# yycho0108/qpwcnet

Hardware: AMD Instinct MI355X
Metric: image-pairs/sec at 256x512 fp32 (higher is better)
Workload: dtype f32; 1 GPU; BASELINE configs[1]: full 6-level PWC-Net (qpwcnet build_flower) inference, batch 8 per GPU, 256x512 fp32, channels_last, d=4 cost volume + WarpV2; global_batch=8, batch_per_gpu=8, parallelism=dp1 (pairs sharded, RCCL all-gather of the 6 per-level EPE), hipgraph=True

## Files before the change

### qpwcnet_amd/csrc/encoder.hip

```cpp
#include "common.h"

namespace qpwc {

__device__ __forceinline__ float enc_mishf(float x) {
    const float e = __builtin_amdgcn_exp2f(fminf(x, 20.0f) * 1.4426950408889634f);
    const float t = e * (e + 2.0f);
    const float m = x * (t * __builtin_amdgcn_rcpf(t + 2.0f));
    return m;
}

typedef float f32x4e __attribute__((ext_vector_type(4)));

__device__ __forceinline__ float2 ld2(const float* p) { return *reinterpret_cast<const float2*>(p); }
__device__ __forceinline__ float2 ld2(const __half* p) { return __half22float2(*reinterpret_cast<const __half2*>(p)); }
__device__ __forceinline__ void st4q(float* p, float4 v) { *reinterpret_cast<float4*>(p) = v; }
__device__ __forceinline__ void st4q(__half* p, float4 v) {
    __half2 lo = __floats2half2_rn(v.x, v.y), hi = __floats2half2_rn(v.z, v.w);
    uint2 u;
    u.x = *reinterpret_cast<unsigned*>(&lo);
    u.y = *reinterpret_cast<unsigned*>(&hi);
    *reinterpret_cast<uint2*>(p) = u;
}

constexpr int kEcTH = 8, kEcTW = 16;
constexpr int kEcHW = kEcTW + 2, kEcNH = (kEcTH + 2) * kEcHW;

template <int C>
__device__ __forceinline__ int ec_slot(int q, int hp) {
    return C == 16 ? (q ^ ((hp >> 2) & 3)) : (q ^ ((hp >> 1) & (C / 4 - 1)));
}

#ifndef QPWC_ENC_NT
#define QPWC_ENC_NT 1
#endif
#ifndef QPWC_UPCONV16_NFB_MIN_WGS
#define QPWC_UPCONV16_NFB_MIN_WGS 512
#endif
#ifndef QPWC_UPCONV256_TH
#define QPWC_UPCONV256_TH 2
#endif
#ifndef QPWC_UPCONV128_TH
#define QPWC_UPCONV128_TH 4
#endif
#ifndef QPWC_UPCONV64_LDS_TOTAL
#define QPWC_UPCONV64_LDS_TOTAL 82944
#endif
#ifndef QPWC_W_NEXT_ALWAYS
#define QPWC_W_NEXT_ALWAYS 1
#endif
#ifndef QPWC_W_NEXT_ALWAYS_F16
#define QPWC_W_NEXT_ALWAYS_F16 0
#endif
#if QPWC_W_NEXT_ALWAYS
#define QPWC_LOAD_W_NEXT(END) load_w(wn, kb + 1 < (END) ? kb + 1 : kb)
#else
#define QPWC_LOAD_W_NEXT(END) do { if (kb + 1 < (END)) load_w(wn, kb + 1); } while (0)
#endif
#ifdef QPWC_ENC_STAMP
__device__ long long g_enc_census[4096 * 6];
#define ENC_CENSUS(i) do { if (census_on) census_p[i] = __builtin_amdgcn_s_memtime(); } while (0)
#else
#define ENC_CENSUS(i) do { } while (0)
#endif
template <int C, int NT>
__global__ __launch_bounds__(256, 4) void conv3x3_mish_kernel(const float* __restrict__ x,
                                                              const float* __restrict__ weight,
                                                              const float* __restrict__ bias,
                                                              float* __restrict__ out, int H, int W,
                                                              int pad_h, int pad_w, int tiles_x, int tiles_y,
                                                              int groups_x) {
    constexpr int NQ = C / 4;
    constexpr int NFT = C / 16;
    constexpr int NKC = C / 16;
    constexpr int NLD = (kEcNH * NQ + 255) / 256;
    constexpr int NBUF = NT > 1 ? 2 : 1;
    __shared__ __attribute__((aligned(16))) float in_s[NBUF * kEcNH * C];
    const int tid0 = threadIdx.x;
    const int wave = __builtin_amdgcn_readfirstlane(tid0 >> 6);
    const int lane = tid0 & 63, n0 = lane & 15, g0 = lane >> 4;
    const int grp = xcd_swizzle(blockIdx.x, gridDim.x);
    const int gx0 = grp % groups_x, ty = (grp / groups_x) % tiles_y, b = grp / (groups_x * tiles_y);
    const int tx0 = gx0 * NT;
    const int Y0 = ty * kEcTH;
    const float* xb = x + (int64_t)b * H * W * C;
    const int Ho = H + pad_h, Wo = W + pad_w;
    float* ob = out + (int64_t)b * Ho * Wo * C;

    auto stage_load = [&](int tid, int tx, float4 (&v)[NLD]) {
        const int X0 = tx * kEcTW;
#pragma unroll
        for (int it = 0; it < NLD; ++it) {
            const int idx = tid + 256 * it;
            const int hp = idx / NQ, q = idx - hp * NQ;
            const int hy = hp / kEcHW, hx = hp - hy * kEcHW;
            const int gy = Y0 - 1 + hy, gx = X0 - 1 + hx;
            v[it] = (idx < kEcNH * NQ && gy >= 0 && gy < H && gx >= 0 && gx < W)
                        ? *reinterpret_cast<const float4*>(xb + ((int64_t)gy * W + gx) * C + 4 * q)
                        : make_float4(0.f, 0.f, 0.f, 0.f);
        }
    };
    auto stage_write = [&](int tid, int buf, const float4 (&v)[NLD]) {
#pragma unroll
        for (int it = 0; it < NLD; ++it) {
            const int idx = tid + 256 * it;
            const int hp = idx / NQ, q = idx - hp * NQ;
            if (idx < kEcNH * NQ)
                *reinterpret_cast<float4*>(in_s + buf * (kEcNH * C) + hp * C + 4 * ec_slot<C>(q, hp)) = v[it];
        }
    };
#ifdef QPWC_ENC_STAMP
    const bool census_on = tid0 == 0 && blockIdx.x < 4096;
    long long* census_p = g_enc_census + (blockIdx.x < 4096 ? blockIdx.x : 0) * 6;
    if (census_on)
        census_p[5] = (long long)(unsigned)__builtin_amdgcn_s_getreg((4) | (0 << 6) | (31 << 11)) |
                      ((long long)(unsigned)__builtin_amdgcn_s_getreg((20) | (0 << 6) | (31 << 11)) << 32);
#endif
    ENC_CENSUS(0);
    float4 st[NLD];
    stage_load(tid0, tx0, st);
#ifdef QPWC_ENC_STAMP
    asm volatile("s_waitcnt vmcnt(0)" ::: "memory");
#endif
    ENC_CENSUS(1);
    stage_write(tid0, 0, st);
    __syncthreads();
    ENC_CENSUS(2);

#pragma unroll 1
    for (int t = 0; t < NT; ++t) {
        const int tx = tx0 + t;
        if (tx >= tiles_x) break;
        const bool more = t + 1 < NT && tx + 1 < tiles_x;

        const int X0 = tx * kEcTW;
        const float* tile_s = in_s + (t & (NBUF - 1)) * (kEcNH * C);
        const float* wt = weight;
        int n = n0, g = g0, tid = tid0;
        if (NT > 1) asm volatile("" : "+r"(wt), "+v"(n), "+v"(g), "+v"(tid));
        if (more) stage_load(tid, tx + 1, st);
#pragma unroll
        for (int ft = 0; ft < NFT; ++ft) {
            f32x4e wld[9][NKC];
#pragma unroll
            for (int k = 0; k < 9; ++k)
#pragma unroll
                for (int kc = 0; kc < NKC; ++kc)
                    wld[k][kc] = *reinterpret_cast<const f32x4e*>(wt + ((int64_t)k * C + 16 * ft + n) * C + 16 * kc + 4 * g);
            f32x4e acc[2];
            acc[0] = f32x4e{0.f, 0.f, 0.f, 0.f};
            acc[1] = f32x4e{0.f, 0.f, 0.f, 0.f};
#pragma unroll
            for (int ky = 0; ky < 3; ++ky)
#pragma unroll
                for (int kx = 0; kx < 3; ++kx)
#pragma unroll
                    for (int kc = 0; kc < NKC; ++kc) {
                        f32x4e bv[2];
#pragma unroll
                        for (int m = 0; m < 2; ++m) {
                            const int hp = (2 * wave + m + ky) * kEcHW + n + kx;
                            const int q = 4 * kc + g;
                            const int slot = ec_slot<C>(q, hp);
                            bv[m] = *reinterpret_cast<const f32x4e*>(tile_s + hp * C + 4 * slot);
                        }
#pragma unroll
                        for (int tt = 0; tt < 4; ++tt)
#pragma unroll
                            for (int m = 0; m < 2; ++m)
                                acc[m] = __builtin_amdgcn_mfma_f32_16x16x4f32(wld[ky * 3 + kx][kc][tt], bv[m][tt], acc[m], 0, 0, 0);
                    }
            if (ft == NFT - 1) ENC_CENSUS(3);
            const float4 bq = *reinterpret_cast<const float4*>(bias + 16 * ft + 4 * g);
#pragma unroll
            for (int m = 0; m < 2; ++m) {
                const int gy = Y0 + 2 * wave + m, gx = X0 + n;
                if (gy < H && gx < W)
                    *reinterpret_cast<float4*>(ob + ((int64_t)gy * Wo + gx) * C + 16 * ft + 4 * g) =
                        make_float4(enc_mishf(acc[m][0] + bq.x), enc_mishf(acc[m][1] + bq.y),
                                    enc_mishf(acc[m][2] + bq.z), enc_mishf(acc[m][3] + bq.w));
            }
        }
        if (pad_w > 0 && X0 + kEcTW >= W) {
            for (int i = tid; i < kEcTH * pad_w * NQ; i += 256) {
                const int q = i % NQ, r = i / NQ, col = r % pad_w, row = r / pad_w;
                const int gy = Y0 + row;
                if (gy < H) *reinterpret_cast<float4*>(ob + ((int64_t)gy * Wo + W + col) * C + 4 * q) = make_float4(0.f, 0.f, 0.f, 0.f);
            }
        }
        if (pad_h > 0 && Y0 + kEcTH >= H) {
            const int x_end = (X0 + kEcTW >= W) ? Wo : X0 + kEcTW;
            for (int i = tid; i < pad_h * (x_end - X0) * NQ; i += 256) {
                const int q = i % NQ, r = i / NQ, col = r % (x_end - X0), row = r / (x_end - X0);
                *reinterpret_cast<float4*>(ob + ((int64_t)(H + row) * Wo + X0 + col) * C + 4 * q) = make_float4(0.f, 0.f, 0.f, 0.f);
            }
        }
// ... 402 lines not shown
    const int tile = xcd_swizzle(blockIdx.x, gridDim.x);
    const int tx = tile % tiles_x, ty = (tile / tiles_x) % tiles_y, b = tile / (tiles_x * tiles_y);
    const int X0 = tx * kEcTW, Y0 = ty * TH;
    const __half* xb = x + (int64_t)b * H * W * C;
    const int Ho = H + pad_h, Wo = W + pad_w;
    __half* ob = out + (int64_t)b * Ho * Wo * C;
    {
        uint4 st[NST];
#pragma unroll
        for (int it = 0; it < NST; ++it) {
            const int idx = tid + 256 * it;
            const int hp = idx / NQ, q = idx - hp * NQ;
            const int hy = hp / HWD, hx = hp - hy * HWD;
            const int gy = Y0 - 1 + hy, gx = X0 - 1 + hx;
            st[it] = (idx < NH * NQ && gy >= 0 && gy < H && gx >= 0 && gx < W)
                         ? *reinterpret_cast<const uint4*>(xb + ((int64_t)gy * W + gx) * C + 8 * q)
                         : make_uint4(0u, 0u, 0u, 0u);
        }
#pragma unroll
        for (int it = 0; it < NST; ++it) {
            const int idx = tid + 256 * it;
            const int hp = idx / NQ, q = idx - hp * NQ;
            if (idx < NH * NQ) *reinterpret_cast<uint4*>(in_s + hp * C + 8 * f16n_slot<C>(q, hp)) = st[it];
        }
    }
    constexpr int NS = C == 16 ? 5 : 9;
    const int gh = C == 16 ? (g >> 1) : 0, gq = C == 16 ? (g & 1) : g;
    f16x8e wv[NS][NFT];
#pragma unroll
    for (int j = 0; j < NS; ++j) {
        const int tap = C == 16 ? 2 * j + gh : j;
#pragma unroll
        for (int ft = 0; ft < NFT; ++ft) {
            wv[j][ft] = f16x8e{0, 0, 0, 0, 0, 0, 0, 0};
            if (tap < 9) wv[j][ft] = *reinterpret_cast<const f16x8e*>(weight + ((int64_t)tap * C + 16 * ft + n) * C + 8 * gq);
        }
    }
    f32x4e acc[RW][NFT];
#pragma unroll
    for (int r = 0; r < RW; ++r)
#pragma unroll
        for (int ft = 0; ft < NFT; ++ft) acc[r][ft] = f32x4e{0.f, 0.f, 0.f, 0.f};
    __syncthreads();
    f16x8e bb[2][RW];
    auto read_b = [&](f16x8e (&bv)[RW], int j) __attribute__((always_inline)) {
        const int t0 = C == 16 ? 2 * j + gh : j;
        const int tap = t0 < 9 ? t0 : 8;
        const int ky = tap / 3, kx = tap - 3 * ky;
#pragma unroll
        for (int r = 0; r < RW; ++r) {
            const int hp = (RW * wave + r + ky) * HWD + n + kx;
            bv[r] = *reinterpret_cast<const f16x8e*>(in_s + hp * C + 8 * f16n_slot<C>(gq, hp));
        }
    };
    read_b(bb[0], 0);
#pragma unroll
    for (int j = 0; j < NS; ++j) {
        if (j + 1 < NS) read_b(bb[(j + 1) & 1], j + 1);
#pragma unroll
        for (int ft = 0; ft < NFT; ++ft)
#pragma unroll
            for (int r = 0; r < RW; ++r)
                acc[r][ft] = __builtin_amdgcn_mfma_f32_16x16x32_f16(wv[j][ft], bb[j & 1][r], acc[r][ft], 0, 0, 0);
        __builtin_amdgcn_sched_barrier(0);
    }
    float4 bqs[NFT];
#pragma unroll
    for (int ft = 0; ft < NFT; ++ft) bqs[ft] = *reinterpret_cast<const float4*>(bias + 16 * ft + 4 * g);
#pragma unroll
    for (int ft = 0; ft < NFT; ++ft) {
        const float4 bq = bqs[ft];
#pragma unroll
        for (int r = 0; r < RW; ++r) {
            const int gy = Y0 + RW * wave + r, gx = X0 + n;
            if (gy < H && gx < W) {
                f16x4e o;
                o[0] = (_Float16)enc_mishf(acc[r][ft][0] + bq.x);
                o[1] = (_Float16)enc_mishf(acc[r][ft][1] + bq.y);
                o[2] = (_Float16)enc_mishf(acc[r][ft][2] + bq.z);
                o[3] = (_Float16)enc_mishf(acc[r][ft][3] + bq.w);
                *reinterpret_cast<f16x4e*>(ob + ((int64_t)gy * Wo + gx) * C + 16 * ft + 4 * g) = o;
            }
        }
    }
    if (pad_w > 0 && X0 + kEcTW >= W) {
        for (int i = tid; i < TH * pad_w * NQ; i += 256) {
            const int q = i % NQ, r = i / NQ, col = r % pad_w, row = r / pad_w;
            const int gy = Y0 + row;
            if (gy < H) *reinterpret_cast<uint4*>(ob + ((int64_t)gy * Wo + W + col) * C + 8 * q) = make_uint4(0u, 0u, 0u, 0u);
        }
    }
    if (pad_h > 0 && Y0 + TH >= H) {
        const int x_end = (X0 + kEcTW >= W) ? Wo : X0 + kEcTW;
        for (int i = tid; i < pad_h * (x_end - X0) * NQ; i += 256) {
            const int q = i % NQ, r = i / NQ, col = r % (x_end - X0), row = r / (x_end - X0);
            *reinterpret_cast<uint4*>(ob + ((int64_t)(H + row) * Wo + X0 + col) * C + 8 * q) = make_uint4(0u, 0u, 0u, 0u);
        }
    }
}

#ifndef QPWC_ENC16_NARROW
#define QPWC_ENC16_NARROW 1
#endif
template <int C>
static int conv3x3_mish_f16_narrow_launch(const void* x, const void* weight, const void* bias, void* out, int B, int H,
                                          int W, int pad_h, int pad_w, hipStream_t s) {
    const int tiles_x = (W + kEcTW - 1) / kEcTW, tiles_y = (H + 15) / 16;
    const int64_t n_tiles = (int64_t)tiles_x * tiles_y * B;
    if (n_tiles > INT32_MAX) {
        set_error("conv3x3_mish_f16: too many tiles");
        return QPWC_E_SHAPE;
    }
    hipLaunchKernelGGL((conv3x3_mish_f16_narrow_kernel<C>), dim3((unsigned)n_tiles), dim3(256), 0, s, (const __half*)x,
                       (const __half*)weight, (const float*)bias, (__half*)out, H, W, pad_h, pad_w, tiles_x, tiles_y);
    return check_launch("conv3x3_mish_f16_narrow_kernel");
}

template <int C, int TH>
static int conv3x3_mish_f16_launch_t(const void* x, const void* weight, const void* bias, void* out, int B, int H,
                                     int W, int pad_h, int pad_w, hipStream_t s) {
    constexpr int NSL = C < 64 ? 1 : C / 64;
    const int tiles_x = (W + kEcTW - 1) / kEcTW, tiles_y = (H + TH - 1) / TH;
    const int64_t n_tiles = (int64_t)tiles_x * tiles_y * B;
    if (n_tiles * NSL > INT32_MAX) {
        set_error("conv3x3_mish_f16: too many tiles");
        return QPWC_E_SHAPE;
    }
    hipLaunchKernelGGL((conv3x3_mish_f16_kernel<C, TH>), dim3((unsigned)(n_tiles * NSL)), dim3(256), 0, s,
                       (const __half*)x, (const __half*)weight, (const float*)bias, (__half*)out, H, W, pad_h, pad_w,
                       tiles_x, tiles_y, (int)n_tiles);
    return check_launch("conv3x3_mish_f16_kernel");
}

int conv3x3_mish_f16_launch(const void* x, const void* weight, const void* bias, void* out, int B, int H, int W,
                            int C, int pad_h, int pad_w, hipStream_t s) {
    switch (C) {
        case 16: return QPWC_ENC16_NARROW ? conv3x3_mish_f16_narrow_launch<16>(x, weight, bias, out, B, H, W, pad_h, pad_w, s)
                                          : conv3x3_mish_f16_launch_t<16, 8>(x, weight, bias, out, B, H, W, pad_h, pad_w, s);
        case 32: return QPWC_ENC16_NARROW ? conv3x3_mish_f16_narrow_launch<32>(x, weight, bias, out, B, H, W, pad_h, pad_w, s)
                                          : conv3x3_mish_f16_launch_t<32, 8>(x, weight, bias, out, B, H, W, pad_h, pad_w, s);
        case 64: return conv3x3_mish_f16_launch_t<64, 8>(x, weight, bias, out, B, H, W, pad_h, pad_w, s);
        case 128: return conv3x3_mish_f16_launch_t<128, 8>(x, weight, bias, out, B, H, W, pad_h, pad_w, s);
        case 256: return conv3x3_mish_f16_launch_t<256, 4>(x, weight, bias, out, B, H, W, pad_h, pad_w, s);
        default: set_error("conv3x3_mish_f16: C=%d not in {16,32,64,128,256}", C); return QPWC_E_SHAPE;
    }
}

struct UpSkip {
    const void* p;
    long long bs, rs, ps;
};

template <int C, int TH>
__global__ __launch_bounds__(256, 2) void upconv4x4s2_mish_kernel(const float* __restrict__ x,
                                                                  const float* __restrict__ weight,
                                                                  const float* __restrict__ bias,
                                                                  float* __restrict__ out, int H, int W, int F,
                                                                  int out_pixel_stride, int tiles_x, int tiles_y,
                                                                  int n_tiles, UpSkip skip) {
    constexpr int NQ = C / 4, NKB = C / 32;
    constexpr int HH = TH + 2, NH = HH * kEcHW;
    constexpr int NST = (NH * NQ + 255) / 256;
    __shared__ __attribute__((aligned(16))) float in_s[NH * C];
    const int tid = threadIdx.x;
    const int wave = __builtin_amdgcn_readfirstlane(tid >> 6);
    const int py = wave >> 1, px = wave & 1;
    const int lane = tid & 63, n = lane & 15, g = lane >> 4;
    const int fblk = blockIdx.x / n_tiles;
    const int tile = xcd_swizzle(blockIdx.x % n_tiles, n_tiles);
    const int tx = tile % tiles_x, ty = (tile / tiles_x) % tiles_y, b = tile / (tiles_x * tiles_y);
    const int X0 = tx * kEcTW, Y0 = ty * TH;
    const int fo = 16 * fblk;
    const float* xb = x + (int64_t)b * H * W * C;
    {
        float4 st[NST];
#pragma unroll
        for (int it = 0; it < NST; ++it) {
            const int idx = tid + 256 * it;
            const int hp = idx / NQ, q = idx - hp * NQ;
            const int hy = hp / kEcHW, hx = hp - hy * kEcHW;
            const int gy = Y0 - 1 + hy, gx = X0 - 1 + hx;
            st[it] = (idx < NH * NQ && gy >= 0 && gy < H && gx >= 0 && gx < W)
                         ? *reinterpret_cast<const float4*>(xb + ((int64_t)gy * W + gx) * C + 4 * q)
                         : make_float4(0.f, 0.f, 0.f, 0.f);
        }
#pragma unroll
        for (int it = 0; it < NST; ++it) {
            const int idx = tid + 256 * it;
            const int hp = idx / NQ, q = idx - hp * NQ;
            if (idx < NH * NQ) *reinterpret_cast<float4*>(in_s + hp * C + 4 * (q ^ (hp & 15))) = st[it];
        }
    }
    const int dy1 = py ? 1 : -1, dx1 = px ? 1 : -1;
    const int ky0 = py ? 2 : 1, ky1 = py ? 0 : 3, kx0 = px ? 2 : 1, kx1 = px ? 0 : 3;
    const int kpos[4] = {ky0 * 4 + kx0, ky0 * 4 + kx1, ky1 * 4 + kx0, ky1 * 4 + kx1};
    const int offy[4] = {0, 0, dy1, dy1}, offx[4] = {0, dx1, 0, dx1};
    f32x4e acc[TH];
#pragma unroll
    for (int m = 0; m < TH; ++m) acc[m] = f32x4e{0.f, 0.f, 0.f, 0.f};
    f32x4e wv[4][2], wn[4][2];
    auto load_w = [&](f32x4e (&w)[4][2], int kb) {
#pragma unroll
        for (int t = 0; t < 4; ++t)
#pragma unroll
            for (int kc = 0; kc < 2; ++kc)
                w[t][kc] = *reinterpret_cast<const f32x4e*>(weight + ((int64_t)kpos[t] * F + fo + n) * C + 32 * kb + 16 * kc + 4 * g);
    };
    load_w(wv, 0);
    __syncthreads();
    auto block = [&](f32x4e (&wv)[4][2], int kb) __attribute__((always_inline)) {
#pragma unroll
        for (int t = 0; t < 4; ++t)
#pragma unroll
            for (int kc = 0; kc < 2; ++kc) {
                f32x4e bv[TH];
#pragma unroll
                for (int m = 0; m < TH; ++m) {
                    const int hp = (m + 1 + offy[t]) * kEcHW + n + 1 + offx[t];
                    bv[m] = *reinterpret_cast<const f32x4e*>(in_s + hp * C + 4 * ((8 * kb + 4 * kc + g) ^ (hp & 15)));
                }
#pragma unroll
                for (int j = 0; j < 4; ++j)
#pragma unroll
                    for (int m = 0; m < TH; ++m)
                        acc[m] = __builtin_amdgcn_mfma_f32_16x16x4f32(wv[t][kc][j], bv[m][j], acc[m], 0, 0, 0);
            }
    };
    static_assert(NKB % 2 == 0, "two blocks per trip");
    if constexpr (QPWC_W_NEXT_ALWAYS && NKB > 2) {
#pragma unroll 1
        for (int kb = 0; kb < NKB; kb += 2) {
            load_w(wn, kb + 1);
            __builtin_amdgcn_sched_barrier(0);
            block(wv, kb);
            load_w(wv, kb + 2 < NKB ? kb + 2 : kb);
            __builtin_amdgcn_sched_barrier(0);
            block(wn, kb + 1);
        }
    } else {
#pragma unroll 1
        for (int kb = 0; kb < NKB; ++kb) {
            if (kb + 1 < NKB) load_w(wn, kb + 1);
            block(wv, kb);
#pragma unroll
            for (int t = 0; t < 4; ++t)
#pragma unroll
                for (int kc = 0; kc < 2; ++kc) wv[t][kc] = wn[t][kc];
        }
    }
    const int H2 = 2 * H, W2 = 2 * W;
    float* ob = out + (int64_t)b * H2 * W2 * out_pixel_stride;
    const float* sk = reinterpret_cast<const float*>(skip.p);
    float4 sv[TH];
    if (sk != nullptr) {
#pragma unroll
        for (int m = 0; m < TH; ++m) {
            const int gy = Y0 + m, gx = X0 + n;
            sv[m] = (gy < H && gx < W)
                        ? *reinterpret_cast<const float4*>(sk + b * skip.bs + (int64_t)(2 * gy + py) * skip.rs +
                                                           (int64_t)(2 * gx + px) * skip.ps + fo + 4 * g)
                        : make_float4(0.f, 0.f, 0.f, 0.f);
        }
    }
    const float4 bq = *reinterpret_cast<const float4*>(bias + fo + 4 * g);
#pragma unroll
    for (int m = 0; m < TH; ++m) {
        const int gy = Y0 + m, gx = X0 + n;
        if (gy < H && gx < W) {
            float* op = ob + ((int64_t)(2 * gy + py) * W2 + 2 * gx + px) * out_pixel_stride + fo + 4 * g;
            *reinterpret_cast<float4*>(op) =
                make_float4(enc_mishf(acc[m][0] + bq.x), enc_mishf(acc[m][1] + bq.y),
                            enc_mishf(acc[m][2] + bq.z), enc_mishf(acc[m][3] + bq.w));
            if (sk != nullptr) *reinterpret_cast<float4*>(op + F) = sv[m];
        }
    }
}

template <int C, int TH>
static int upconv_launch_t(const void* x, const void* weight, const void* bias, void* out, int B, int H, int W, int F,
                           int out_pixel_stride, hipStream_t s, UpSkip skip) {
    const int tiles_x = (W + kEcTW - 1) / kEcTW, tiles_y = (H + TH - 1) / TH;
    const int64_t n_tiles = (int64_t)tiles_x * tiles_y * B;
    if (n_tiles * (F / 16) > INT32_MAX) {
        set_error("upconv4x4s2_mish: too many tiles");
        return QPWC_E_SHAPE;
    }
    constexpr size_t kStatic = (size_t)(TH + 2) * kEcHW * C * sizeof(float);
    const size_t want = (C == 64 && QPWC_UPCONV64_LDS_TOTAL && n_tiles * (F / 16) <= 2048) ? QPWC_UPCONV64_LDS_TOTAL : 0;
    const size_t extra = want > kStatic ? want - kStatic : 0;
    hipLaunchKernelGGL((upconv4x4s2_mish_kernel<C, TH>), dim3((unsigned)(n_tiles * (F / 16))), dim3(256), extra, s,
                       (const float*)x, (const float*)weight, (const float*)bias, (float*)out, H, W, F,
                       out_pixel_stride, tiles_x, tiles_y, (int)n_tiles, skip);
    return check_launch("upconv4x4s2_mish_kernel");
}

int upconv4x4s2_mish_launch(const void* x, const void* weight, const void* bias, void* out, int B, int H, int W, int C,
                            int F, int out_pixel_stride, hipStream_t s, const void* skip, int64_t skip_bs, int64_t skip_rs,
                            int64_t skip_ps) {
    const UpSkip sk{skip, (long long)skip_bs, (long long)skip_rs, (long long)skip_ps};
    switch (C) {
        case 64: return upconv_launch_t<64, 8>(x, weight, bias, out, B, H, W, F, out_pixel_stride, s, sk);
        case 128: return upconv_launch_t<128, QPWC_UPCONV128_TH>(x, weight, bias, out, B, H, W, F, out_pixel_stride, s, sk);
        case 256: return upconv_launch_t<256, QPWC_UPCONV256_TH>(x, weight, bias, out, B, H, W, F, out_pixel_stride, s, sk);
        default: set_error("upconv4x4s2_mish: C=%d not in {64,128,256}", C); return QPWC_E_SHAPE;
    }
}

template <int C, int TH>
__global__ __launch_bounds__(256, 2) void upconv4x4s2_mish_f16_kernel(const __half* __restrict__ x,
                                                                      const __half* __restrict__ weight,
                                                                      const float* __restrict__ bias,
                                                                      __half* __restrict__ out, int H, int W, int F,
                                                                      int out_pixel_stride, int tiles_x, int tiles_y,
                                                                      int n_tiles, UpSkip skip, int nfb) {
    constexpr int NQ = C / 8, NKB = C / 32;
    constexpr int HH = TH + 2, NH = HH * kEcHW;
    constexpr int NST = (NH * NQ + 255) / 256;
    __shared__ __attribute__((aligned(16))) __half in_s[NH * C];
    const int tid = threadIdx.x;
    const int wave = __builtin_amdgcn_readfirstlane(tid >> 6);
    const int py = wave >> 1, px = wave & 1;
    const int lane = tid & 63, n = lane & 15, g = lane >> 4;
    const int fblk0 = (blockIdx.x / n_tiles) * nfb;
    const int tile = xcd_swizzle(blockIdx.x % n_tiles, n_tiles);
    const int tx = tile % tiles_x, ty = (tile / tiles_x) % tiles_y, b = tile / (tiles_x * tiles_y);
    const int X0 = tx * kEcTW, Y0 = ty * TH;
    int fo = 16 * fblk0;
    const __half* xb = x + (int64_t)b * H * W * C;
    {
        uint4 st[NST];
#pragma unroll
        for (int it = 0; it < NST; ++it) {
            const int idx = tid + 256 * it;
            const int hp = idx / NQ, q = idx - hp * NQ;
            const int hy = hp / kEcHW, hx = hp - hy * kEcHW;
            const int gy = Y0 - 1 + hy, gx = X0 - 1 + hx;
            st[it] = (idx < NH * NQ && gy >= 0 && gy < H && gx >= 0 && gx < W)
                         ? *reinterpret_cast<const uint4*>(xb + ((int64_t)gy * W + gx) * C + 8 * q)
                         : make_uint4(0u, 0u, 0u, 0u);
        }
#pragma unroll
        for (int it = 0; it < NST; ++it) {
            const int idx = tid + 256 * it;
            const int hp = idx / NQ, q = idx - hp * NQ;
            if (idx < NH * NQ) *reinterpret_cast<uint4*>(in_s + hp * C + 8 * f16_slot<C>(q, hp)) = st[it];
        }
    }
    const int dy1 = py ? 1 : -1, dx1 = px ? 1 : -1;
    const int ky0 = py ? 2 : 1, ky1 = py ? 0 : 3, kx0 = px ? 2 : 1, kx1 = px ? 0 : 3;
    const int kpos[4] = {ky0 * 4 + kx0, ky0 * 4 + kx1, ky1 * 4 + kx0, ky1 * 4 + kx1};
    const int offy[4] = {0, 0, dy1, dy1}, offx[4] = {0, dx1, 0, dx1};
    f32x4e acc[TH];
    f16x8e wv[4], wn[4];
    auto load_w = [&](f16x8e (&w)[4], int kb) {
#pragma unroll
        for (int t = 0; t < 4; ++t)
            w[t] = *reinterpret_cast<const f16x8e*>(weight + ((int64_t)kpos[t] * F + fo + n) * C + 32 * kb + 8 * g);
    };
    load_w(wv, 0);
    __syncthreads();
    auto block = [&](f16x8e (&wv)[4], int kb) __attribute__((always_inline)) {
#pragma unroll
        for (int t = 0; t < 4; ++t)
#pragma unroll
            for (int m = 0; m < TH; ++m) {
                const int hp = (m + 1 + offy[t]) * kEcHW + n + 1 + offx[t];
                const f16x8e bv = *reinterpret_cast<const f16x8e*>(in_s + hp * C + 8 * f16_slot<C>(4 * kb + g, hp));
                acc[m] = __builtin_amdgcn_mfma_f32_16x16x32_f16(wv[t], bv, acc[m], 0, 0, 0);
            }
    };
#pragma unroll 1
    for (int fb = 0; fb < nfb; ++fb) {
    fo = 16 * (fblk0 + fb);
    if (fb > 0) load_w(wv, 0);
#pragma unroll
    for (int m = 0; m < TH; ++m) acc[m] = f32x4e{0.f, 0.f, 0.f, 0.f};
#if QPWC_W_NEXT_ALWAYS_F16
    {
        int kb = 0;
#pragma unroll 1
        for (; kb + 1 < NKB; kb += 2) {
            load_w(wn, kb + 1);
            __builtin_amdgcn_sched_barrier(0);
            block(wv, kb);
            load_w(wv, kb + 2 < NKB ? kb + 2 : kb);
            __builtin_amdgcn_sched_barrier(0);
            block(wn, kb + 1);
        }
        if (kb < NKB) block(wv, kb);
    }
#else
#pragma unroll 1
    for (int kb = 0; kb < NKB; ++kb) {
        if (kb + 1 < NKB) load_w(wn, kb + 1);
        block(wv, kb);
#pragma unroll
        for (int t = 0; t < 4; ++t) wv[t] = wn[t];
    }
#endif
    const int H2 = 2 * H, W2 = 2 * W;
    __half* ob = out + (int64_t)b * H2 * W2 * out_pixel_stride;
    const __half* sk = reinterpret_cast<const __half*>(skip.p);
    f16x4e sv[TH];
    if (sk != nullptr) {
#pragma unroll
        for (int m = 0; m < TH; ++m) {
            const int gy = Y0 + m, gx = X0 + n;
            sv[m] = (gy < H && gx < W)
                        ? *reinterpret_cast<const f16x4e*>(sk + b * skip.bs + (int64_t)(2 * gy + py) * skip.rs +
                                                           (int64_t)(2 * gx + px) * skip.ps + fo + 4 * g)
                        : f16x4e{0, 0, 0, 0};
        }
    }
    const float4 bq = *reinterpret_cast<const float4*>(bias + fo + 4 * g);
#pragma unroll
    for (int m = 0; m < TH; ++m) {
        const int gy = Y0 + m, gx = X0 + n;
        if (gy < H && gx < W) {
            f16x4e o;
            o[0] = (_Float16)enc_mishf(acc[m][0] + bq.x);
            o[1] = (_Float16)enc_mishf(acc[m][1] + bq.y);
            o[2] = (_Float16)enc_mishf(acc[m][2] + bq.z);
            o[3] = (_Float16)enc_mishf(acc[m][3] + bq.w);
            __half* op = ob + ((int64_t)(2 * gy + py) * W2 + 2 * gx + px) * out_pixel_stride + fo + 4 * g;
            *reinterpret_cast<f16x4e*>(op) = o;
            if (sk != nullptr) *reinterpret_cast<f16x4e*>(op + F) = sv[m];
        }
    }
    }
}

template <int C, int TH>
static int upconv_f16_launch_t(const void* x, const void* weight, const void* bias, void* out, int B, int H, int W, int F,
                               int out_pixel_stride, hipStream_t s, UpSkip skip) {
    const int tiles_x = (W + kEcTW - 1) / kEcTW, tiles_y = (H + TH - 1) / TH;
    const int64_t n_tiles = (int64_t)tiles_x * tiles_y * B;
    if (n_tiles * (F / 16) > INT32_MAX) {
        set_error("upconv4x4s2_mish_f16: too many tiles");
        return QPWC_E_SHAPE;
    }
    int nfb = 1;
    while (nfb * 2 <= F / 16 && (F / 16) % (nfb * 2) == 0 && n_tiles * (F / 16) / (nfb * 2) >= QPWC_UPCONV16_NFB_MIN_WGS) nfb *= 2;
    hipLaunchKernelGGL((upconv4x4s2_mish_f16_kernel<C, TH>), dim3((unsigned)(n_tiles * (F / 16) / nfb)), dim3(256), 0, s,
                       (const __half*)x, (const __half*)weight, (const float*)bias, (__half*)out, H, W, F,
                       out_pixel_stride, tiles_x, tiles_y, (int)n_tiles, skip, nfb);
    return check_launch("upconv4x4s2_mish_f16_kernel");
}

int upconv4x4s2_mish_f16_launch(const void* x, const void* weight, const void* bias, void* out, int B, int H, int W,
                                int C, int F, int out_pixel_stride, hipStream_t s, const void* skip, int64_t skip_bs,
                                int64_t skip_rs, int64_t skip_ps) {
    const UpSkip sk{skip, (long long)skip_bs, (long long)skip_rs, (long long)skip_ps};
    switch (C) {
        case 64: return upconv_f16_launch_t<64, 8>(x, weight, bias, out, B, H, W, F, out_pixel_stride, s, sk);
        case 128: return upconv_f16_launch_t<128, 8>(x, weight, bias, out, B, H, W, F, out_pixel_stride, s, sk);
        case 256: return upconv_f16_launch_t<256, 4>(x, weight, bias, out, B, H, W, F, out_pixel_stride, s, sk);
// ... 521 lines not shown
```

Baseline: 7325 pairs/s.

## Rewrite fp32 upconv4x4s2 kernel with async LDS ring for halo and weight streaming

Result: no change. 7319 pairs/s (-0.1%).

```diff
diff --git a/qpwcnet_amd/csrc/encoder.hip b/qpwcnet_amd/csrc/encoder.hip
--- a/qpwcnet_amd/csrc/encoder.hip
+++ b/qpwcnet_amd/csrc/encoder.hip
@@ -35,12 +35,6 @@
 #endif
 #ifndef QPWC_UPCONV16_NFB_MIN_WGS
 #define QPWC_UPCONV16_NFB_MIN_WGS 512
-#endif
-#ifndef QPWC_UPCONV256_TH
-#define QPWC_UPCONV256_TH 2
-#endif
-#ifndef QPWC_UPCONV128_TH
-#define QPWC_UPCONV128_TH 4
 #endif
 #ifndef QPWC_UPCONV64_LDS_TOTAL
 #define QPWC_UPCONV64_LDS_TOTAL 82944
@@ -749,16 +743,31 @@
 };
 
 template <int C, int TH>
-__global__ __launch_bounds__(256, 2) void upconv4x4s2_mish_kernel(const float* __restrict__ x,
-                                                                  const float* __restrict__ weight,
-                                                                  const float* __restrict__ bias,
-                                                                  float* __restrict__ out, int H, int W, int F,
-                                                                  int out_pixel_stride, int tiles_x, int tiles_y,
-                                                                  int n_tiles, UpSkip skip) {
-    constexpr int NQ = C / 4, NKB = C / 32;
-    constexpr int HH = TH + 2, NH = HH * kEcHW;
-    constexpr int NST = (NH * NQ + 255) / 256;
-    __shared__ __attribute__((aligned(16))) float in_s[NH * C];
+struct UrShape {
+    static constexpr int NKB = C / 32;
+    static constexpr int NS = 4 * NKB;
+    static constexpr int KU = TH >= 8 ? 1 : 2;
+    static constexpr int UPS = 2 / KU;
+    static constexpr int SLOTS = TH >= 8 ? 4 : 5;
+    static constexpr int NH = (TH + 2) * kEcHW;
+    static constexpr int NHI = (NH * 8 + 255) / 256;
+    static constexpr int HBLK = 4 * NHI * 1024;
+    static constexpr int WBASE = 2 * HBLK;
+    static constexpr int LDS = WBASE + 4 * SLOTS * 2048;
+    static_assert(NKB % 2 == 0, "the K-loop walks pairs of 32-channel blocks");
+    static_assert(SLOTS >= 4 && 2 * (SLOTS - 3) + NHI <= 12 && 2 * (SLOTS - 2) <= 12, "ew_wait_vm's counts");
+    static_assert(LDS <= 80 * 1024, "a decoder workgroup must fit beside a 79-80 KB flow-chain workgroup on a CU");
+};
+
+template <int C, int TH>
+__global__ __launch_bounds__(256, 2) void upconv4x4s2_mish_ring_kernel(const float* __restrict__ x,
+                                                                       const float* __restrict__ weight,
+                                                                       const float* __restrict__ bias,
+                                                                       float* __restrict__ out, int H, int W, int F,
+                                                                       int out_pixel_stride, int tiles_x, int tiles_y,
+                                                                       int n_tiles, UpSkip skip) {
+    using S = UrShape<C, TH>;
+    __shared__ __attribute__((aligned(1024))) char smem[S::LDS];
     const int tid = threadIdx.x;
     const int wave = __builtin_amdgcn_readfirstlane(tid >> 6);
     const int py = wave >> 1, px = wave & 1;
@@ -768,98 +777,132 @@
     const int tx = tile % tiles_x, ty = (tile / tiles_x) % tiles_y, b = tile / (tiles_x * tiles_y);
     const int X0 = tx * kEcTW, Y0 = ty * TH;
     const int fo = 16 * fblk;
-    const float* xb = x + (int64_t)b * H * W * C;
-    {
-        float4 st[NST];
-#pragma unroll
-        for (int it = 0; it < NST; ++it) {
-            const int idx = tid + 256 * it;
-            const int hp = idx / NQ, q = idx - hp * NQ;
-            const int hy = hp / kEcHW, hx = hp - hy * kEcHW;
-            const int gy = Y0 - 1 + hy, gx = X0 - 1 + hx;
-            st[it] = (idx < NH * NQ && gy >= 0 && gy < H && gx >= 0 && gx < W)
-                         ? *reinterpret_cast<const float4*>(xb + ((int64_t)gy * W + gx) * C + 4 * q)
-                         : make_float4(0.f, 0.f, 0.f, 0.f);
-        }
-#pragma unroll
-        for (int it = 0; it < NST; ++it) {
-            const int idx = tid + 256 * it;
-            const int hp = idx / NQ, q = idx - hp * NQ;
-            if (idx < NH * NQ) *reinterpret_cast<float4*>(in_s + hp * C + 4 * (q ^ (hp & 15))) = st[it];
-        }
-    }
+    const __amdgpu_buffer_rsrc_t rx = __builtin_amdgcn_make_buffer_rsrc(
+        const_cast<float*>(x) + (int64_t)b * H * W * C, 0, H * W * C * 4, 0x00020000);
+    const __amdgpu_buffer_rsrc_t rw = __builtin_amdgcn_make_buffer_rsrc(const_cast<float*>(weight), 0, 16 * F * C * 4, 0x00020000);
+
+    unsigned hoff[S::NHI];
+#pragma unroll
+    for (int j = 0; j < S::NHI; ++j) {
+        const int i = (wave * S::NHI + j) * 64 + lane;
+        const int hp = i >> 3, q = (i & 7) ^ (hp & 7);
+        const int hy = hp / kEcHW, hx = hp - hy * kEcHW;
+        const int gy = Y0 - 1 + hy, gx = X0 - 1 + hx;
+        hoff[j] = (hp < S::NH && gy >= 0 && gy < H && gx >= 0 && gx < W) ? (unsigned)(((gy * W + gx) * C + 4 * q) * 4) : kEwOob;
+    }
+    const unsigned woff = (unsigned)(((fo + n) * C + 4 * g) * 4);
     const int dy1 = py ? 1 : -1, dx1 = px ? 1 : -1;
     const int ky0 = py ? 2 : 1, ky1 = py ? 0 : 3, kx0 = px ? 2 : 1, kx1 = px ? 0 : 3;
-    const int kpos[4] = {ky0 * 4 + kx0, ky0 * 4 + kx1, ky1 * 4 + kx0, ky1 * 4 + kx1};
-    const int offy[4] = {0, 0, dy1, dy1}, offx[4] = {0, dx1, 0, dx1};
+    const int slab = F * C * 4;
+    const int kofs[4] = {(ky0 * 4 + kx0) * slab, (ky0 * 4 + kx1) * slab, (ky1 * 4 + kx0) * slab, (ky1 * 4 + kx1) * slab};
+    const int toff[4] = {0, dx1, dy1 * kEcHW, dy1 * kEcHW + dx1};
+    auto issue_h = [&](int kb) __attribute__((always_inline)) {
+#pragma unroll
+        for (int j = 0; j < S::NHI; ++j)
+            ew_dma16(rx, smem + (kb & 1) * S::HBLK + (wave * S::NHI + j) * 1024, hoff[j], kb * 128);
+    };
+    auto issue_w = [&](int kb, int tap, int slot) __attribute__((always_inline)) {
+        char* dst = smem + S::WBASE + (slot * 4 + wave) * 2048;
+#pragma unroll
+        for (int kc = 0; kc < 2; ++kc)
+            ew_dma16(rw, dst + kc * 1024, woff, kofs[tap] + (32 * kb + 16 * kc) * 4);
+    };
+    f32x4e wa[2][S::KU], pb[2][S::KU][TH];
+    auto read = [&](int hslot, int tap, int wslot, int kc0, int buf) __attribute__((always_inline)) {
+        const char* ws = smem + S::WBASE + (wslot * 4 + wave) * 2048 + lane * 16;
+        const char* hs = smem + hslot * S::HBLK;
+#pragma unroll
+        for (int k = 0; k < S::KU; ++k) {
+            const int kc = kc0 + k;
+            wa[buf][k] = *reinterpret_cast<const f32x4e*>(ws + kc * 1024);
+#pragma unroll
+            for (int m = 0; m < TH; ++m) {
+                const int hp = (m + 1) * kEcHW + 1 + n + toff[tap];
+                pb[buf][k][m] = *reinterpret_cast<const f32x4e*>(hs + hp * 128 + 16 * ((4 * kc + g) ^ (hp & 7)));
+            }
+        }
+    };
     f32x4e acc[TH];
 #pragma unroll
-    for (int m = 0; m < TH; ++m) acc[m] = f32x4e{0.f, 0.f, 0.f, 0.f};
-    f32x4e wv[4][2], wn[4][2];
-    auto load_w = [&](f32x4e (&w)[4][2], int kb) {
-#pragma unroll
-        for (int t = 0; t < 4; ++t)
-#pragma unroll
-            for (int kc = 0; kc < 2; ++kc)
-                w[t][kc] = *reinterpret_cast<const f32x4e*>(weight + ((int64_t)kpos[t] * F + fo + n) * C + 32 * kb + 16 * kc + 4 * g);
-    };
-    load_w(wv, 0);
-    __syncthreads();
-    auto block = [&](f32x4e (&wv)[4][2], int kb) __attribute__((always_inline)) {
-#pragma unroll
-        for (int t = 0; t < 4; ++t)
-#pragma unroll
-            for (int kc = 0; kc < 2; ++kc) {
-                f32x4e bv[TH];
-#pragma unroll
-                for (int m = 0; m < TH; ++m) {
-                    const int hp = (m + 1 + offy[t]) * kEcHW + n + 1 + offx[t];
-                    bv[m] = *reinterpret_cast<const f32x4e*>(in_s + hp * C + 4 * ((8 * kb + 4 * kc + g) ^ (hp & 15)));
+    for (int m = 0; m < TH; ++m) {
+        acc[m] = f32x4e{0.f, 0.f, 0.f, 0.f};
+        ew_pin_agpr(acc[m]);
+    }
+    const int H2 = 2 * H, W2 = 2 * W;
+    const float* sk = reinterpret_cast<const float*>(skip.p);
+    float4 sv[TH], bq;
+
+    issue_h(0);
+#pragma unroll
+    for (int s = 0; s < S::SLOTS - 1; ++s) issue_w(s >> 2, s & 3, s);
+    ew_wait_vm(2 * (S::SLOTS - 2));
+    __builtin_amdgcn_s_barrier();
+    read(0, 0, 0, 0, 0);
+
+    auto pair = [&](int p, const bool LAST) __attribute__((always_inline)) {
+#pragma unroll
+        for (int t = 0; t < 8; ++t) {
+#pragma unroll
+            for (int h = 0; h < S::UPS; ++h) {
+                const int u = t * S::UPS + h;
+                const bool step_end = h == S::UPS - 1;
+                const bool more = !(LAST && t == 7 && step_end);
+                if (step_end) {
+                    if (more) {
+                        const int tb = t & 3;
+                        const bool h_out = tb >= 1 && !(LAST && t >= 4);
+                        const int cw = 2 * (S::SLOTS - 3) + (h_out && tb <= S::SLOTS - 2 ? S::NHI : 0);
+                        const int ch = 2 * (tb - 1);
+                        ew_wait_vm(tb == 3 && h_out && ch < cw ? ch : cw);
+                        if (tb == 3) {
+                            asm volatile("s_waitcnt lgkmcnt(0)" ::: "memory");
+                            __builtin_amdgcn_s_barrier();
+                        }
+                    }
+                    {
+                        const int c = t + S::SLOTS - 1;
+                        const bool past = LAST && c >= 8;
+                        issue_w(past ? S::NKB - 1 : 2 * p + (c >> 2), past ? 3 : (c & 3), (8 * p + c) % S::SLOTS);
+                    }
+                    if (t == 0) issue_h(2 * p + 1);
+                    if (t == 4 && !LAST) issue_h(2 * p + 2);
                 }
-#pragma unroll
-                for (int j = 0; j < 4; ++j)
-#pragma unroll
-                    for (int m = 0; m < TH; ++m)
-                        acc[m] = __builtin_amdgcn_mfma_f32_16x16x4f32(wv[t][kc][j], bv[m][j], acc[m], 0, 0, 0);
+                if (more) {
+                    if (step_end) read(((t + 1) >> 2) & 1, (t + 1) & 3, (8 * p + t + 1) % S::SLOTS, 0, (u + 1) & 1);
+                    else read((t >> 2) & 1, t & 3, (8 * p + t) % S::SLOTS, (h + 1) * S::KU, (u + 1) & 1);
+                } else {
+                    if (sk != nullptr) {
+#pragma unroll
+                        for (int m = 0; m < TH; ++m) {
+                            const int gy = Y0 + m, gx = X0 + n;
+                            sv[m] = (gy < H && gx < W)
+                                        ? *reinterpret_cast<const float4*>(sk + b * skip.bs + (int64_t)(2 * gy + py) * skip.rs +
+                                                                           (int64_t)(2 * gx + px) * skip.ps + fo + 4 * g)
+                                        : make_float4(0.f, 0.f, 0.f, 0.f);
+                        }
+                    }
+                    bq = *reinterpret_cast<const float4*>(bias + fo + 4 * g);
+                }
+                __builtin_amdgcn_sched_barrier(0);
+#pragma unroll
+                for (int k = 0; k < S::KU; ++k)
+#pragma unroll
+                    for (int j = 0; j < 4; ++j)
+#pragma unroll
+                        for (int m = 0; m < TH; ++m)
+                            acc[m] = __builtin_amdgcn_mfma_f32_16x16x4f32(wa[u & 1][k][j], pb[u & 1][k][m][j], acc[m], 0, 0, 0);
+#pragma unroll
+                for (int m = 0; m < TH; ++m) ew_pin_agpr(acc[m]);
+                __builtin_amdgcn_sched_barrier(0);
             }
-    };
-    static_assert(NKB % 2 == 0, "two blocks per trip");
-    if constexpr (QPWC_W_NEXT_ALWAYS && NKB > 2) {
+        }
+    };
 #pragma unroll 1
-        for (int kb = 0; kb < NKB; kb += 2) {
-            load_w(wn, kb + 1);
-            __builtin_amdgcn_sched_barrier(0);
-            block(wv, kb);
-            load_w(wv, kb + 2 < NKB ? kb + 2 : kb);
-            __builtin_amdgcn_sched_barrier(0);
-            block(wn, kb + 1);
-        }
-    } else {
-#pragma unroll 1
-        for (int kb = 0; kb < NKB; ++kb) {
-            if (kb + 1 < NKB) load_w(wn, kb + 1);
-            block(wv, kb);
-#pragma unroll
-            for (int t = 0; t < 4; ++t)
-#pragma unroll
-                for (int kc = 0; kc < 2; ++kc) wv[t][kc] = wn[t][kc];
-        }
-    }
-    const int H2 = 2 * H, W2 = 2 * W;
+    for (int p = 0; p < S::NKB / 2 - 1; ++p) pair(p, false);
+    pair(S::NKB / 2 - 1, true);
+    asm volatile("s_waitcnt vmcnt(0)" ::: "memory");
+
     float* ob = out + (int64_t)b * H2 * W2 * out_pixel_stride;
-    const float* sk = reinterpret_cast<const float*>(skip.p);
-    float4 sv[TH];
-    if (sk != nullptr) {
-#pragma unroll
-        for (int m = 0; m < TH; ++m) {
-            const int gy = Y0 + m, gx = X0 + n;
-            sv[m] = (gy < H && gx < W)
-                        ? *reinterpret_cast<const float4*>(sk + b * skip.bs + (int64_t)(2 * gy + py) * skip.rs +
-                                                           (int64_t)(2 * gx + px) * skip.ps + fo + 4 * g)
-                        : make_float4(0.f, 0.f, 0.f, 0.f);
-        }
-    }
-    const float4 bq = *reinterpret_cast<const float4*>(bias + fo + 4 * g);
 #pragma unroll
     for (int m = 0; m < TH; ++m) {
         const int gy = Y0 + m, gx = X0 + n;
@@ -878,17 +921,17 @@
                            int out_pixel_stride, hipStream_t s, UpSkip skip) {
     const int tiles_x = (W + kEcTW - 1) / kEcTW, tiles_y = (H + TH - 1) / TH;
     const int64_t n_tiles = (int64_t)tiles_x * tiles_y * B;
-    if (n_tiles * (F / 16) > INT32_MAX) {
-        set_error("upconv4x4s2_mish: too many tiles");
+    if (n_tiles * (F / 16) > INT32_MAX || (int64_t)H * W * C * 4 > INT32_MAX || (int64_t)16 * F * C * 4 > INT32_MAX) {
+        set_error("upconv4x4s2_mish: too many tiles, or a frame or a weight tensor of 2 GiB or more");
         return QPWC_E_SHAPE;
     }
-    constexpr size_t kStatic = (size_t)(TH + 2) * kEcHW * C * sizeof(float);
+    constexpr size_t kStatic = UrShape<C, TH>::LDS;
     const size_t want = (C == 64 && QPWC_UPCONV64_LDS_TOTAL && n_tiles * (F / 16) <= 2048) ? QPWC_UPCONV64_LDS_TOTAL : 0;
     const size_t extra = want > kStatic ? want - kStatic : 0;
-    hipLaunchKernelGGL((upconv4x4s2_mish_kernel<C, TH>), dim3((unsigned)(n_tiles * (F / 16))), dim3(256), extra, s,
+    hipLaunchKernelGGL((upconv4x4s2_mish_ring_kernel<C, TH>), dim3((unsigned)(n_tiles * (F / 16))), dim3(256), extra, s,
                        (const float*)x, (const float*)weight, (const float*)bias, (float*)out, H, W, F,
                        out_pixel_stride, tiles_x, tiles_y, (int)n_tiles, skip);
-    return check_launch("upconv4x4s2_mish_kernel");
+    return check_launch("upconv4x4s2_mish_ring_kernel");
 }
 
 int upconv4x4s2_mish_launch(const void* x, const void* weight, const void* bias, void* out, int B, int H, int W, int C,
@@ -897,8 +940,8 @@
     const UpSkip sk{skip, (long long)skip_bs, (long long)skip_rs, (long long)skip_ps};
     switch (C) {
         case 64: return upconv_launch_t<64, 8>(x, weight, bias, out, B, H, W, F, out_pixel_stride, s, sk);
-        case 128: return upconv_launch_t<128, QPWC_UPCONV128_TH>(x, weight, bias, out, B, H, W, F, out_pixel_stride, s, sk);
-        case 256: return upconv_launch_t<256, QPWC_UPCONV256_TH>(x, weight, bias, out, B, H, W, F, out_pixel_stride, s, sk);
+        case 128: return upconv_launch_t<128, 4>(x, weight, bias, out, B, H, W, F, out_pixel_stride, s, sk);
+        case 256: return upconv_launch_t<256, 2>(x, weight, bias, out, B, H, W, F, out_pixel_stride, s, sk);
         default: set_error("upconv4x4s2_mish: C=%d not in {64,128,256}", C); return QPWC_E_SHAPE;
     }
 }
```
